# cisco-open/flame

Measured on AMD Instinct MI355X. Metric: aggregated params/sec (device-resident), 1024-client FedAvg @1/2/4/8 GPU, higher is better.
Workload: dtype f32

## Files before the change

### flame_amd/csrc/fedagg.hip

```cpp
#include <hip/hip_runtime.h>
#include <hip/hip_fp16.h>

#include <atomic>
#include <cstdint>
#include <cstdio>
#include <cstring>
#include <cstdarg>
#include <type_traits>

#include "../../include/flame_amd.h"
#include "fastmath.h"

#if defined(__FAST_MATH__) || (defined(__FINITE_MATH_ONLY__) && __FINITE_MATH_ONLY__)
#error "fedagg.hip must not be built with -ffast-math / -ffinite-math-only"
#endif

namespace {

constexpr int kBlock = 256;
#ifndef FLAME_T_CLIENT_UNROLL
#define FLAME_T_CLIENT_UNROLL 8
#endif
constexpr int kClientUnroll = FLAME_T_CLIENT_UNROLL;
#ifndef FLAME_T_CLIENT_UNROLL16
#define FLAME_T_CLIENT_UNROLL16 8
#endif
constexpr int kClientUnroll16 = FLAME_T_CLIENT_UNROLL16;
#ifndef FLAME_T_LO_UNROLL
#define FLAME_T_LO_UNROLL 3
#endif
constexpr int kLoUnroll = FLAME_T_LO_UNROLL;
#ifndef FLAME_T_LO_UNROLL16
#define FLAME_T_LO_UNROLL16 4
#endif
constexpr int kLoUnroll16 = FLAME_T_LO_UNROLL16;
#ifndef FLAME_T_LO_LDS
#define FLAME_T_LO_LDS 65536
#endif
constexpr int kLoLds = FLAME_T_LO_LDS;
#ifndef FLAME_T_LO_WGC
#define FLAME_T_LO_WGC 8
#endif
constexpr int kLoWGC = FLAME_T_LO_WGC;
#ifndef FLAME_T_LO_BURST_MAX_CLIENTS
#define FLAME_T_LO_BURST_MAX_CLIENTS 512
#endif
constexpr int kLoBurstMaxClients = FLAME_T_LO_BURST_MAX_CLIENTS;
constexpr int kLoHeld = kLoWGC > 1 ? kLoWGC * 4096 : 0;
constexpr int kLoDynLds = kLoLds > kLoHeld ? kLoLds - kLoHeld : 0;
#ifndef FLAME_T_LO_MIN_CLIENTS
#define FLAME_T_LO_MIN_CLIENTS 64
#endif
constexpr int kLoMinClients = FLAME_T_LO_MIN_CLIENTS;
#ifndef FLAME_T_LO_MIN_CHUNKS
#define FLAME_T_LO_MIN_CHUNKS 4096
#endif
constexpr int64_t kLoMinChunks = FLAME_T_LO_MIN_CHUNKS;
#ifndef FLAME_T_OPT_WGC
#define FLAME_T_OPT_WGC 4
#endif
constexpr int kOptWGC = FLAME_T_OPT_WGC;
#ifndef FLAME_T_OPT_UNROLL
#define FLAME_T_OPT_UNROLL 3
#endif
constexpr int kOptUnroll = FLAME_T_OPT_UNROLL;
#ifndef FLAME_T_HB
#define FLAME_T_HB 8
#endif
constexpr int kHB = FLAME_T_HB;
#ifndef FLAME_T_HIER_UNROLL16
#define FLAME_T_HIER_UNROLL16 4
#endif
constexpr int kHierUnroll16 = FLAME_T_HIER_UNROLL16;
#ifndef FLAME_T_HBL
#define FLAME_T_HBL 16
#endif
constexpr int kHBL = FLAME_T_HBL;
#ifndef FLAME_T_HIER_LDS_UNROLL16
#define FLAME_T_HIER_LDS_UNROLL16 6
#endif
constexpr int kHierLdsUnroll16 = FLAME_T_HIER_LDS_UNROLL16;
#ifndef FLAME_T_HLDS_MIN_MIDS
#define FLAME_T_HLDS_MIN_MIDS 16
#endif
constexpr int kHLdsMinMids = FLAME_T_HLDS_MIN_MIDS;
#ifndef FLAME_T_HLO_UNROLL
#define FLAME_T_HLO_UNROLL 3
#endif
constexpr int kHLoUnroll = FLAME_T_HLO_UNROLL;
#ifndef FLAME_T_HLO_MIN_CLIENTS
#define FLAME_T_HLO_MIN_CLIENTS 64
#endif
constexpr int kHLoMinClients = FLAME_T_HLO_MIN_CLIENTS;
#ifndef FLAME_T_HLO_MIN_CHUNKS
#define FLAME_T_HLO_MIN_CHUNKS 4096
#endif
constexpr int64_t kHLoMinChunks = FLAME_T_HLO_MIN_CHUNKS;
#ifndef FLAME_T_HLO_LDS_F32
#define FLAME_T_HLO_LDS_F32 65536
#endif
constexpr int kHLoLdsF32 = FLAME_T_HLO_LDS_F32;
#ifndef FLAME_T_HLO_LDS16
#define FLAME_T_HLO_LDS16 53248
#endif
constexpr int kHLoLds16 = FLAME_T_HLO_LDS16;
#ifndef FLAME_T_DYN_UNROLL
#define FLAME_T_DYN_UNROLL 4
#endif
constexpr int kDynUnroll = FLAME_T_DYN_UNROLL;
#ifndef FLAME_T_CHAIN_UNROLL
#define FLAME_T_CHAIN_UNROLL 16
#endif
constexpr int kChainUnroll = FLAME_T_CHAIN_UNROLL;
#ifndef FLAME_T_CHAIN_UNROLL16
#define FLAME_T_CHAIN_UNROLL16 8
#endif
constexpr int kChainUnroll16 = FLAME_T_CHAIN_UNROLL16;
#ifndef FLAME_T_CHAIN_LDS
#define FLAME_T_CHAIN_LDS 53248
#endif
constexpr int kChainLds = FLAME_T_CHAIN_LDS;
#ifndef FLAME_T_BF16_PACKED
#define FLAME_T_BF16_PACKED 1
#endif
constexpr bool kBf16Packed = FLAME_T_BF16_PACKED != 0;
#ifndef FLAME_T_F16_PACKED
#define FLAME_T_F16_PACKED 1
#endif
constexpr bool kF16Packed = FLAME_T_F16_PACKED != 0;
#ifndef FLAME_T_F16_HWROOT
#define FLAME_T_F16_HWROOT 1
#endif
constexpr bool kF16HwRoot = FLAME_T_F16_HWROOT != 0;
#ifndef FLAME_T_F16_NATIVE
#define FLAME_T_F16_NATIVE 1
#endif
constexpr bool kF16Native = FLAME_T_F16_NATIVE != 0;
#ifndef FLAME_T_F16_HSQRT
#define FLAME_T_F16_HSQRT 1
#endif
constexpr bool kF16HalfRoot = FLAME_T_F16_HSQRT != 0;
#ifndef FLAME_T_HALF_ADMIT
#define FLAME_T_HALF_ADMIT 1
#endif
constexpr bool kHalfAdmit = FLAME_T_HALF_ADMIT != 0;
#ifndef FLAME_T_YOGI_SIGN
#define FLAME_T_YOGI_SIGN 1
#endif
constexpr bool kYogiSelect = FLAME_T_YOGI_SIGN != 0;
constexpr int kEwBlock = 256;

thread_local char g_err[512] = "";

int set_err(int code, const char* fmt, ...) {
    va_list ap;
    va_start(ap, fmt);
    vsnprintf(g_err, sizeof(g_err), fmt, ap);
    va_end(ap);
    return code;
}

int check_launch(const char* what) {
    hipError_t e = hipGetLastError();
    if (e != hipSuccess) return set_err(FLAME_EHIP, "%s: %s", what, hipGetErrorString(e));
    g_err[0] = 0;
    return FLAME_OK;
}

__device__ __forceinline__ float bf16_round(float x) {
    return static_cast<float>(static_cast<__bf16>(x));
}
__device__ __forceinline__ float bf16_to_f32(uint16_t b) {
    return __uint_as_float(static_cast<uint32_t>(b) << 16);
}
__device__ __forceinline__ uint16_t f32_to_bf16_exact(float x) {
    return static_cast<uint16_t>(__float_as_uint(x) >> 16);
}
__device__ __forceinline__ float bf16_rnd1(float x) {
    float r;
    asm("v_cvt_pk_bf16_f32 %0, 0, %1" : "=v"(r) : "v"(x));
    return r;
}
using f2 = __attribute__((ext_vector_type(2))) float;
__device__ __forceinline__ f2 bf16_rnd2(f2 x) { return f2{bf16_rnd1(x.x), bf16_rnd1(x.y)}; }
__device__ __forceinline__ f2 splat2(float x) { return f2{x, x}; }
__device__ __forceinline__ float f16_round(float x) {
    asm volatile("" : "+v"(x));
    return static_cast<float>(static_cast<_Float16>(x));
}
__device__ __forceinline__ float f16_to_f32(uint16_t h) {
    _Float16 v;
    __builtin_memcpy(&v, &h, 2);
    return static_cast<float>(v);
}
__device__ __forceinline__ uint16_t f32_to_f16_bits(float x) {
    asm volatile("" : "+v"(x));
    _Float16 v = static_cast<_Float16>(x);
    uint16_t h;
    __builtin_memcpy(&h, &v, 2);
    return h;
}
__device__ __forceinline__ f2 f16_rnd2(f2 x) {
    uint32_t p;
    asm("v_cvt_pk_f16_f32 %0, %1, %2" : "=v"(p) : "v"(x.x), "v"(x.y));
    return f2{f16_to_f32(static_cast<uint16_t>(p)), f16_to_f32(static_cast<uint16_t>(p >> 16))};
}

using h2 = __attribute__((ext_vector_type(2))) _Float16;
using us2 = __attribute__((ext_vector_type(2))) unsigned short;
__device__ __forceinline__ h2 h2_of(uint32_t u) { return __builtin_bit_cast(h2, u); }
__device__ __forceinline__ uint32_t u_of(h2 h) { return __builtin_bit_cast(uint32_t, h); }
__device__ __forceinline__ f2 widen_h2(uint32_t u) {
    const h2 h = h2_of(u);
    return f2{static_cast<float>(h.x), static_cast<float>(h.y)};
}
__device__ __forceinline__ uint32_t smul_h2(float s, uint32_t x, float& lo, float& hi) {
    uint32_t r;
    asm("v_fma_mix_f32 %0, %1, %2, neg(0) op_sel_hi:[0,1,0]" : "=v"(lo) : "s"(s), "v"(x));
    asm("v_fma_mix_f32 %0, %1, %2, neg(0) op_sel:[0,1,0] op_sel_hi:[0,1,0]" : "=v"(hi) : "s"(s), "v"(x));
    asm("v_cvt_pk_f16_f32 %0, %1, %2" : "=v"(r) : "v"(lo), "v"(hi));
    return r;
}
__device__ __forceinline__ uint32_t smul_h2(float s, uint32_t x) {
    float lo, hi;
    return smul_h2(s, x, lo, hi);
}
template <int HI>
__device__ __forceinline__ float div_rn_h(uint32_t x, float den) {
    const float y = flame_fm::rcp_rn(den);
    float q0;
    if constexpr (HI) asm("v_fma_mix_f32 %0, %1, %2, neg(0) op_sel:[0,1,0] op_sel_hi:[0,1,0]" : "=v"(q0) : "v"(y), "v"(x));
    else asm("v_fma_mix_f32 %0, %1, %2, neg(0) op_sel_hi:[0,1,0]" : "=v"(q0) : "v"(y), "v"(x));
    const float a = static_cast<float>(HI ? h2_of(x).y : h2_of(x).x);
    const float rn = __builtin_fmaf(den, q0, -a);
    return __builtin_fmaf(-rn, y, q0);
}
__device__ __forceinline__ uint32_t pk_h2(f2 x) {
    uint32_t r;
    asm("v_cvt_pk_f16_f32 %0, %1, %2" : "=v"(r) : "v"(x.x), "v"(x.y));
    return r;
}
__device__ __forceinline__ h2 sign_h2(h2 x) {
    const h2 z = x + h2{0, 0};
    const h2 big = (z * h2{65504, 65504}) * h2{65504, 65504};
    return __builtin_elementwise_max(__builtin_elementwise_min(big, h2{1, 1}), h2{-1, -1});
}

template <int DT> struct Tr;

template <> struct Tr<FLAME_F32> {
    using T = float; using A = float; static constexpr int EPT = 4;
    __device__ static A ld(T x) { return x; }
    __device__ static T st(A a) { return a; }
    __device__ static A tmp(T v, float r, double) { return __fmul_rn(v, r); }
    __device__ static A mulr(A a, float r, double) { return __fmul_rn(a, r); }
    __device__ static A add(A a, A t) { return __fadd_rn(a, t); }
};
template <> struct Tr<FLAME_BF16> {
    using T = uint16_t; using A = float; static constexpr int EPT = 8;
    __device__ static A ld(T x) { return bf16_to_f32(x); }
    __device__ static T st(A a) { return f32_to_bf16_exact(a); }
    __device__ static A tmp(T v, float r, double) { return bf16_round(__fmul_rn(bf16_to_f32(v), r)); }
// ... 2247 lines not shown
                    for (int j = 0; j < EPT; ++j) {
                        S::op(w[j], X::st(acc[j]), g, static_cast<double>(g), &d[j]);
                        const A t = X::tmp(d[j], rt, 0.0);
                        top[j] = have_top ? X::add(top[j], t) : t;
                    }
                }
                if constexpr (HL) held[u * kBlock + threadIdx.x] = pack<T, EPT>(w);
                else pend[u] = pack<T, EPT>(w);
                if (dp) st_v(dp, pack<T, EPT>(d));
            }
            have_top = true;
            }
            if (!(flags & FLAME_HIER_MID_READONLY)) {
#pragma unroll
                for (int u = 0; u < HB; ++u) {
                    if (u >= nb) break;
                    T* wp = mid_ptr(m0 + u);
                    V16 pv;
                    if constexpr (HL) pv = held[u * kBlock + threadIdx.x];
                    else pv = pend[u];
                    st_v(wp, pv);
                }
            }
        }
        T o[EPT];
#pragma unroll
        for (int j = 0; j < EPT; ++j) o[j] = X::st(top[j]);
        if (sg.top_agg_out) st_v(reinterpret_cast<T*>(sg.top_agg_out) + e0, pack<T, EPT>(o));
        if (flags & FLAME_HIER_TOP_APPLY) {
            T* gp = reinterpret_cast<T*>(sg.top_w) + e0;
            T gw[EPT];
            unpack<T, EPT>(ld_v(gp), gw);
#pragma unroll
            for (int j = 0; j < EPT; ++j) S::op(gw[j], o[j], top_goal, static_cast<double>(top_goal), nullptr);
            st_v(gp, pack<T, EPT>(gw));
        }
        return;
    }
    hier_tail<DT, SYNC>(sg, e0, coff, wrow, drow, crow, mid_ptr, n_mids, n_clients, mid_rates, mid_goal, top_rates,
                        top_goal, flags);
}

template <int DT, int CU, bool SYNC, int HB, bool HL>
__global__ __launch_bounds__(kBlock) void hier_fedbuff_kernel(const flame_hier_segment* __restrict__ segs, int n_segs,
                                                    int n_mids, int n_clients, const uint64_t* __restrict__ mid_w,
                                                    const uint64_t* __restrict__ mid_delta,
                                                    const uint64_t* __restrict__ clients,
                                                    const float* __restrict__ mid_rates,
                                                    const float* __restrict__ mid_goal,
                                                    const float* __restrict__ top_rates, float top_goal,
                                                    unsigned flags) {
    hier_fedbuff_body<DT, CU, SYNC, HB, HL>(segs, n_segs, n_mids, n_clients, mid_w, mid_delta, clients, mid_rates, mid_goal,
                                    top_rates, top_goal, flags);
}

template <int DT, int CU, bool SYNC, int HB, bool HL>
__global__ __launch_bounds__(kBlock) void hier_fedbuff_kernel_argmeta(const ArgMeta meta, int n_segs, int n_mids, int n_clients,
                                                            int o_mid_w, int o_mid_delta, int o_clients,
                                                            int o_mid_rates, int o_mid_goal, int o_top_rates,
                                                            float top_goal, unsigned flags) {
    (void)sizeof(meta);
    const uint64_t* w = (const uint64_t*)__builtin_amdgcn_kernarg_segment_ptr();
    hier_fedbuff_body<DT, CU, SYNC, HB, HL>(reinterpret_cast<const flame_hier_segment*>(w), n_segs, n_mids, n_clients,
                                    w + o_mid_w, o_mid_delta >= 0 ? w + o_mid_delta : nullptr, w + o_clients,
                                    reinterpret_cast<const float*>(w + o_mid_rates),
                                    reinterpret_cast<const float*>(w + o_mid_goal),
                                    reinterpret_cast<const float*>(w + o_top_rates), top_goal, flags);
}
#pragma clang diagnostic pop

template <int DT, int CU, bool VEC>
__device__ __forceinline__ void feddyn_chunk(const flame_dyn_segment& sg, const uint64_t* __restrict__ row,
                                             const uint32_t* __restrict__ sflags, int n_steps, int n_phase1,
                                             float ra32, float rm32, double ra64, double rm64, int64_t e0,
                                             int64_t coff, int64_t hoff) {
    using X = Tr<DT>;
    using T = typename X::T;
    using A = typename X::A;
    constexpr int EPT = X::EPT;
    const int64_t ooff = e0 * static_cast<int64_t>(sizeof(T));
    auto load = [&](uint64_t base, int64_t off, T (&x)[EPT]) {
        const T* p = reinterpret_cast<const T*>(reinterpret_cast<const char*>(base) + off);
        if constexpr (VEC) {
            unpack<T, EPT>(ld_nt(p), x);
        } else {
#pragma unroll
            for (int j = 0; j < EPT; ++j) x[j] = (e0 + j < sg.numel) ? ld1(p + j) : T(0);
        }
    };
    auto store = [&](void* base, int64_t off, const T (&x)[EPT]) {
        T* p = reinterpret_cast<T*>(reinterpret_cast<char*>(base) + off);
        if constexpr (VEC) {
            st_v(p, pack<T, EPT>(x));
        } else {
#pragma unroll
            for (int j = 0; j < EPT; ++j)
                if (e0 + j < sg.numel) st1(p + j, x[j]);
        }
    };
    A avg[EPT], mean[EPT];
    {
        T b[EPT];
        load(reinterpret_cast<uint64_t>(sg.in), ooff, b);
#pragma unroll
        for (int j = 0; j < EPT; ++j) { avg[j] = X::ld(b[j]); mean[j] = A(0); }
    }
#pragma unroll 1
    for (int phase = 0; phase < 2; ++phase) {
        const int end = phase ? n_steps : n_phase1;
#pragma unroll 1
        for (int k = phase ? n_phase1 : 0; k < end; k += CU) {
            const int nb = (end - k < CU) ? end - k : CU;
            T w[CU][EPT], h[CU][EPT];
#pragma unroll
            for (int u = 0; u < CU; ++u) {
                if (u >= nb) break;
                const uint32_t f = sflags[k + u];
                const uint64_t* p = row + static_cast<int64_t>(k + u) * 3;
                if (f & FLAME_DYN_W) load(p[0], coff, w[u]);
                if (f & FLAME_DYN_HIN) load(p[1], hoff, h[u]);
            }
#pragma unroll
            for (int u = 0; u < CU; ++u) {
                if (u >= nb) break;
                const uint32_t f = sflags[k + u];
                if (f & FLAME_DYN_AVG) {
#pragma unroll
                    for (int j = 0; j < EPT; ++j) avg[j] = X::add(avg[j], X::tmp(w[u][j], ra32, ra64));
                }
                if (f & FLAME_DYN_HOUT) {
                    if (f & FLAME_DYN_HIN) {
#pragma unroll
                        for (int j = 0; j < EPT; ++j) h[u][j] = X::st(X::add(X::ld(h[u][j]), X::ld(w[u][j])));
                    } else {
#pragma unroll
                        for (int j = 0; j < EPT; ++j) h[u][j] = w[u][j];
                    }
                    store(reinterpret_cast<void*>(row[static_cast<int64_t>(k + u) * 3 + 2]), hoff, h[u]);
                }
                if (f & FLAME_DYN_MEAN) {
#pragma unroll
                    for (int j = 0; j < EPT; ++j) mean[j] = X::add(mean[j], X::tmp(h[u][j], rm32, rm64));
                }
            }
        }
    }
    T o[EPT], c[EPT];
#pragma unroll
    for (int j = 0; j < EPT; ++j) { o[j] = X::st(avg[j]); c[j] = X::st(X::add(avg[j], mean[j])); }
    store(sg.out, ooff, o);
    store(sg.cld, ooff, c);
}

template <int DT, int CU>
__global__ __launch_bounds__(kBlock) void feddyn_kernel(const flame_dyn_segment* __restrict__ segs, int n_segs,
                                                        const uint64_t* __restrict__ steps,
                                                        const uint32_t* __restrict__ sflags, int n_steps,
                                                        int n_phase1, float ra32, float rm32, double ra64,
                                                        double rm64) {
    using X = Tr<DT>;
    constexpr int EPT = X::EPT;
    const int64_t chunk = xcd_slot(blockIdx.x, gridDim.x);
    const int s = find_segment(segs, n_segs, chunk);
    const flame_dyn_segment sg = segs[s];
    const int64_t e0 = (chunk - sg.chunk_begin) * chunk_elems<DT>() + static_cast<int64_t>(threadIdx.x) * EPT;
    if (e0 >= sg.numel) return;
    const int64_t coff = client_offset<DT>(sg, chunk);
    const int64_t hoff = sg.hist_tile_stride
        ? (chunk - sg.chunk_begin) * sg.hist_tile_stride + static_cast<int64_t>(threadIdx.x) * EPT * static_cast<int64_t>(sizeof(typename X::T))
        : e0 * static_cast<int64_t>(sizeof(typename X::T));
    const uint64_t* row = steps + static_cast<int64_t>(s) * n_steps * 3;
    const bool vec = (e0 + EPT <= sg.numel) && !(sg.flags & FLAME_SEG_UNALIGNED);
    if (vec)
        feddyn_chunk<DT, CU, true>(sg, row, sflags, n_steps, n_phase1, ra32, rm32, ra64, rm64, e0, coff, hoff);
    else
        feddyn_chunk<DT, 1, false>(sg, row, sflags, n_steps, n_phase1, ra32, rm32, ra64, rm64, e0, coff, hoff);
}

__host__ __device__ __forceinline__ uint64_t mix64(uint64_t z) {
    z = (z ^ (z >> 30)) * 0xBF58476D1CE4E5B9ull;
    z = (z ^ (z >> 27)) * 0x94D049BB133111EBull;
    return z ^ (z >> 31);
}

template <int DT>
__global__ __launch_bounds__(kEwBlock) void synth_kernel(void* out, int64_t numel, uint64_t ck, int64_t start, float scale) {
    const int64_t stride = static_cast<int64_t>(gridDim.x) * kEwBlock;
    for (int64_t j = static_cast<int64_t>(blockIdx.x) * kEwBlock + threadIdx.x; j < numel; j += stride) {
        const uint64_t h = mix64(ck + static_cast<uint64_t>(start + j) * 0x9E3779B97F4A7C15ull);
        const int32_t s = static_cast<int32_t>((h & 0xFFFFu) + ((h >> 16) & 0xFFFFu) + ((h >> 32) & 0xFFFFu) + (h >> 48)) - 131070;
        const float x = __fmul_rn(static_cast<float>(s), scale);
        if constexpr (DT == FLAME_F32) st1(reinterpret_cast<float*>(out) + j, x);
        else if constexpr (DT == FLAME_BF16) st1(reinterpret_cast<uint16_t*>(out) + j, f32_to_bf16_exact(bf16_round(x)));
        else st1(reinterpret_cast<uint16_t*>(out) + j, f32_to_f16_bits(x));
    }
}

__device__ __forceinline__ void philox4x32_10(uint32_t (&c)[4], uint32_t k0, uint32_t k1) {
#pragma unroll
    for (int r = 0; r < 10; ++r) {
        const uint64_t p0 = 0xD2511F53ull * c[0], p1 = 0xCD9E8D57ull * c[2];
        const uint32_t n0 = static_cast<uint32_t>(p1 >> 32) ^ c[1] ^ k0;
        const uint32_t n2 = static_cast<uint32_t>(p0 >> 32) ^ c[3] ^ k1;
        c[0] = n0; c[1] = static_cast<uint32_t>(p1); c[2] = n2; c[3] = static_cast<uint32_t>(p0);
        k0 += 0x9E3779B9u; k1 += 0xBB67AE85u;
    }
}

__device__ __forceinline__ float noise_neg2ln(float u) {
    const uint32_t bits = __float_as_uint(u);
    int e = static_cast<int>(bits >> 23) - 127;
    float m = __uint_as_float((bits & 0x7FFFFFu) | 0x3F800000u);
    if (m > 0x1.6a09e6p+0f) { m = __fmul_rn(m, 0.5f); e += 1; }
    const float f = __fadd_rn(m, -1.0f);
    const float s = __fdiv_rn(f, __fadd_rn(f, 2.0f));
    const float z = __fmul_rn(s, s);
    float p = 0x1.745d18p-4f;
    p = __fadd_rn(__fmul_rn(p, z), 0x1.c71c72p-4f);
    p = __fadd_rn(__fmul_rn(p, z), 0x1.24924ap-3f);
    p = __fadd_rn(__fmul_rn(p, z), 0x1.99999ap-3f);
    p = __fadd_rn(__fmul_rn(p, z), 0x1.555556p-2f);
    p = __fmul_rn(p, z);
    const float t = __fadd_rn(s, s);
    const float lg = __fadd_rn(t, __fmul_rn(t, p));
    const float ef = static_cast<float>(e);
    const float ln = __fadd_rn(__fmul_rn(ef, 0x1.62e4p-1f), __fadd_rn(lg, __fmul_rn(ef, 0x1.7f7d1cp-20f)));
    return __fmul_rn(-2.0f, ln);
}

__device__ __forceinline__ void noise_sincos(uint32_t k, float& co, float& si) {
    const uint32_t o = k >> 21, j = k & 0x1FFFFFu;
    const uint32_t jj = (o & 1u) ? 0x200000u - j : j;
    const float phi = __fmul_rn(static_cast<float>(jj), 0x1.921fb6p-22f);
    const float z = __fmul_rn(phi, phi);
    float ps = 0x1.71de3ap-19f;
    ps = __fadd_rn(__fmul_rn(ps, z), -0x1.a01a02p-13f);
    ps = __fadd_rn(__fmul_rn(ps, z), 0x1.111112p-7f);
    ps = __fadd_rn(__fmul_rn(ps, z), -0x1.555556p-3f);
    const float s = __fadd_rn(phi, __fmul_rn(__fmul_rn(phi, z), ps));
    float pc = -0x1.27e4fcp-22f;
    pc = __fadd_rn(__fmul_rn(pc, z), 0x1.a01a02p-16f);
    pc = __fadd_rn(__fmul_rn(pc, z), -0x1.6c16c2p-10f);
    pc = __fadd_rn(__fmul_rn(pc, z), 0x1.555556p-5f);
    pc = __fadd_rn(__fmul_rn(pc, z), -0x1p-1f);
    const float c = __fadd_rn(1.0f, __fmul_rn(z, pc));
    const bool swap = ((o + 1u) >> 1) & 1u, cneg = ((o + 2u) >> 2) & 1u, sneg = o >> 2;
    const float c0 = swap ? s : c, s0 = swap ? c : s;
    co = __uint_as_float(__float_as_uint(c0) ^ (cneg ? 0x80000000u : 0u));
    si = __uint_as_float(__float_as_uint(s0) ^ (sneg ? 0x80000000u : 0u));
}

__device__ __forceinline__ void noise_pair(uint32_t xu, uint32_t xk, float& ze, float& zo) {
    const uint64_t v = 2ull * xu + 1ull;
    const float hi = static_cast<float>(static_cast<uint32_t>(v >> 17));
    const float lo = static_cast<float>(static_cast<uint32_t>(v & 0x1FFFFu));
    const float u = __fmul_rn(__fadd_rn(__fmul_rn(hi, 131072.0f), lo), 0x1p-33f);
    const float r = __builtin_sqrtf(noise_neg2ln(u));
    float co, si;
    noise_sincos(xk >> 8, co, si);
    ze = __fmul_rn(r, co);
    zo = __fmul_rn(r, si);
}

__device__ __forceinline__ void noise_block(uint32_t k0, uint32_t k1, uint32_t round, uint32_t stream, uint64_t b,
                                            float (&z)[4]) {
    uint32_t c[4] = {static_cast<uint32_t>(b), static_cast<uint32_t>(b >> 32), stream, round};
    philox4x32_10(c, k0, k1);
    noise_pair(c[0], c[1], z[0], z[1]);
    noise_pair(c[2], c[3], z[2], z[3]);
}

template <int DT>
__device__ __forceinline__ typename Tr<DT>::T noise_value(float z, float std32, double std64) {
    if constexpr (DT == FLAME_F64) return __dmul_rn(static_cast<double>(z), std64);
    else if constexpr (DT == FLAME_F32) return __fmul_rn(z, std32);
    else if constexpr (DT == FLAME_BF16) return f32_to_bf16_exact(bf16_round(__fmul_rn(z, std32)));
    else return f32_to_f16_bits(__fmul_rn(z, std32));
}

template <int DT>
__global__ __launch_bounds__(kBlock) void noise_fill_kernel(const flame_segment* __restrict__ segs, int n_segs,
                                                          const uint32_t* __restrict__ streams,
                                                          const int64_t* __restrict__ starts, uint32_t k0, uint32_t k1,
                                                          uint32_t round, float std32, double std64) {
    using T = typename Tr<DT>::T;
    constexpr int EPT = Tr<DT>::EPT;
    const int64_t chunk = blockIdx.x;
    const int s = find_segment(segs, n_segs, chunk);
    const flame_segment sg = segs[s];
    const int64_t e0 = (chunk - sg.chunk_begin) * chunk_elems<DT>() + static_cast<int64_t>(threadIdx.x) * EPT;
    if (e0 >= sg.numel) return;
    const uint32_t stream = streams[s];
    const uint64_t start = static_cast<uint64_t>(starts[s]);
    const uint64_t g0 = start + static_cast<uint64_t>(e0);
    T* op = reinterpret_cast<T*>(sg.out) + e0;
    float z[4];
    if ((e0 + EPT <= sg.numel) && !(sg.flags & FLAME_SEG_UNALIGNED) && !(start & 3u)) {
        T x[EPT];
        if constexpr (EPT >= 4) {
#pragma unroll
            for (int q = 0; q < EPT / 4; ++q) {
                noise_block(k0, k1, round, stream, (g0 >> 2) + q, z);
#pragma unroll
                for (int j = 0; j < 4; ++j) x[4 * q + j] = noise_value<DT>(z[j], std32, std64);
            }
        } else {
            noise_block(k0, k1, round, stream, g0 >> 2, z);
            const bool up = g0 & 2u;
            x[0] = noise_value<DT>(up ? z[2] : z[0], std32, std64);
            x[1] = noise_value<DT>(up ? z[3] : z[1], std32, std64);
        }
        st_v(op, pack<T, EPT>(x));
        return;
    }
    uint64_t have = ~0ull;
    for (int j = 0; j < EPT; ++j) {
        if (e0 + j >= sg.numel) break;
        const uint64_t g = g0 + static_cast<uint64_t>(j);
        if ((g >> 2) != have) {
            have = g >> 2;
            noise_block(k0, k1, round, stream, have, z);
        }
        const uint32_t l = static_cast<uint32_t>(g) & 3u;
        const float zl = l == 0 ? z[0] : l == 1 ? z[1] : l == 2 ? z[2] : z[3];
        st1(op + j, noise_value<DT>(zl, std32, std64));
// ... 867 lines not shown
                               n_segs, cl, n_clients, rates32, step_end, flags, b1, omb1, b2, omb2, eta, tau);
        });
    });
    if (!known) return set_err(FLAME_ENOTSUP, "%s: dtype %d not supported (f32, bf16, f16)", who, dtype);
    return launched(BR_CHAIN + dtype * 3 + variant, who);
}

int flame_fedopt_reduce_adapt_f64(int variant, unsigned flags, const flame_segment* segs, int32_t n_segs,
                                  int64_t n_chunks, const void* const* clients, int32_t n_clients,
                                  const double* rates64, double b1, double omb1, double b2, double omb2, double eta,
                                  double tau, void* stream) {
    const char* const who = "flame_fedopt_reduce_adapt_f64";
    if (int rc = validate(segs, n_segs, n_chunks, n_clients, clients)) return rc;
    if (n_clients > 0 && !rates64) return set_err(FLAME_EINVAL, "rate array is NULL");
    if (int rc = check_variant(who, variant)) return rc;
    if (int rc = check_flags(who, flags, kOptFlags)) return rc;
    hipStream_t st = reinterpret_cast<hipStream_t>(stream);
    const dim3 grid(static_cast<unsigned>(n_chunks)), block(kBlock);
    auto cl = reinterpret_cast<const uint64_t*>(clients);
    const Hyper64 h{b1, omb1, b2, omb2, eta, tau};
    dispatch_variant(variant, [&](auto vr) {
        hipLaunchKernelGGL((fedopt_kernel_f64<decltype(vr)::value, kClientUnroll>), grid, block, 0, st, segs, n_segs, cl,
                           n_clients, rates64, flags, h, n_chunks);
    });
    return launched(BR_OPT_F64 + variant, who);
}

int flame_fedopt_chain_f64(int variant, unsigned flags, const flame_segment* segs, int32_t n_segs, int64_t n_chunks,
                           const void* const* clients, int32_t n_clients, const double* rates64,
                           const uint8_t* step_end, double b1, double omb1, double b2, double omb2, double eta,
                           double tau, void* stream) {
    const char* const who = "flame_fedopt_chain_f64";
    if (int rc = validate(segs, n_segs, n_chunks, n_clients, clients)) return rc;
    if (n_clients < 1 || !rates64 || !step_end)
        return set_err(FLAME_EINVAL, "%s: needs >= 1 client, a rate array and a step_end array", who);
    if (int rc = check_variant(who, variant)) return rc;
    if (int rc = check_flags(who, flags, FLAME_OPT_STATE_ZERO)) return rc;
    hipStream_t st = reinterpret_cast<hipStream_t>(stream);
    const dim3 grid(static_cast<unsigned>(n_chunks)), block(kBlock);
    auto cl = reinterpret_cast<const uint64_t*>(clients);
    const Hyper64 h{b1, omb1, b2, omb2, eta, tau};
    dispatch_variant(variant, [&](auto vr) {
        hipLaunchKernelGGL((fedopt_chain_kernel_f64<decltype(vr)::value, kClientUnroll>), grid, block, 0, st, segs, n_segs,
                           cl, n_clients, rates64, step_end, flags, h);
    });
    return launched(BR_CHAIN_F64 + variant, who);
}

int flame_fedopt_reduce_adapt_argmeta(int dtype, int variant, unsigned flags, const void* host_meta,
                                      int64_t meta_bytes, int32_t n_segs, int64_t n_chunks, int32_t n_clients,
                                      int64_t off_clients, int64_t off_r32, float b1, float omb1, float b2,
                                      float omb2, float eta, float tau, void* stream) {
    const char* const who = "flame_fedopt_reduce_adapt_argmeta";
    ArgMeta m;
    if (int rc = load_argmeta(who, host_meta, meta_bytes, m)) return rc;
    if (n_segs <= 0 || n_clients < 0) return set_err(FLAME_EINVAL, "%s: n_segs <= 0 or n_clients < 0", who);
    if (int rc = check_chunks(n_chunks)) return rc;
    if (int rc = check_flags(who, flags, kOptFlags)) return rc;
    if (int rc = check_variant(who, variant)) return rc;
    if (static_cast<int64_t>(n_segs) * static_cast<int64_t>(sizeof(flame_segment)) > meta_bytes ||
        !inside(meta_bytes, off_clients, static_cast<int64_t>(n_segs) * n_clients * 8) ||
        (n_clients > 0 && !inside(meta_bytes, off_r32, static_cast<int64_t>(n_clients) * 4)))
        return set_err(FLAME_EINVAL, "%s: a table lies outside the metadata block", who);
    const OptArgMeta src{&m, static_cast<int>(off_clients / 8), n_clients > 0 ? static_cast<int>(off_r32 / 8) : -1};
    return launch_opt(who, dtype, variant, flags, src, n_segs, n_clients, n_chunks, Hyper32{b1, omb1, b2, omb2, eta, tau},
                      stream);
}

int flame_fedbuff_scale_add(int dtype, const flame_segment* segs, int32_t n_segs, int64_t n_chunks, int64_t goal,
                            void* stream) {
    if (int rc = validate(segs, n_segs, n_chunks, 0, nullptr)) return rc;
    if (goal == 0) return set_err(FLAME_EINVAL, "agg_goal must be nonzero");
    hipStream_t st = reinterpret_cast<hipStream_t>(stream);
    const dim3 grid(static_cast<unsigned>(n_chunks)), block(kEwBlock);
    const float gf = static_cast<float>(goal);
    const double gd = static_cast<double>(goal);
    const bool known = dispatch<FLAME_F32, FLAME_F64, FLAME_BF16, FLAME_F16>(dtype, [&](auto dt) {
        hipLaunchKernelGGL((scale_add_kernel<decltype(dt)::value>), grid, block, 0, st, segs, n_segs, gf, gd);
    });
    if (!known)
        return set_err(FLAME_ENOTSUP, "flame_fedbuff_scale_add: dtype %d not supported (integer tensors raise in the reference)", dtype);
    return launched(BR_SA + dtype, "flame_fedbuff_scale_add");
}

int flame_hier_fedbuff(int dtype, unsigned flags, const flame_hier_segment* segs, int32_t n_segs, int64_t n_chunks,
                       int32_t n_mids, int32_t n_clients, const void* const* mid_w, const void* const* mid_delta,
                       const void* const* clients, const float* mid_rates, const float* mid_goal,
                       const float* top_rates, float top_goal, void* stream) {
    const char* const who = "flame_hier_fedbuff";
    if (!segs || n_segs <= 0) return set_err(FLAME_EINVAL, "segment table is NULL or n_segs <= 0");
    if (int rc = check_chunks(n_chunks)) return rc;
    if (n_mids < 1 || n_clients < 1) return set_err(FLAME_EINVAL, "%s: need >= 1 middle and >= 1 arrival per middle", who);
    if (!mid_w || !clients || !mid_rates || !mid_goal || !top_rates) return set_err(FLAME_EINVAL, "%s: NULL table", who);
    if (int rc = check_hier_flags(who, flags, top_goal)) return rc;
    const HierTables src{segs, reinterpret_cast<const uint64_t*>(mid_w), reinterpret_cast<const uint64_t*>(mid_delta),
                         reinterpret_cast<const uint64_t*>(clients), mid_rates, mid_goal, top_rates};
    return launch_hier(who, dtype, flags, src, n_segs, n_chunks, n_mids, n_clients, top_goal, stream);
}

int flame_hier_fedbuff_argmeta(int dtype, unsigned flags, const void* host_meta, int64_t meta_bytes, int32_t n_segs,
                               int64_t n_chunks, int32_t n_mids, int32_t n_clients, int64_t off_mid_w,
                               int64_t off_mid_delta, int64_t off_clients, int64_t off_mid_rates,
                               int64_t off_mid_goal, int64_t off_top_rates, float top_goal, void* stream) {
    const char* const who = "flame_hier_fedbuff_argmeta";
    ArgMeta m;
    if (int rc = load_argmeta(who, host_meta, meta_bytes, m)) return rc;
    if (n_segs <= 0) return set_err(FLAME_EINVAL, "segment table is empty");
    if (int rc = check_chunks(n_chunks)) return rc;
    if (n_mids < 1 || n_clients < 1) return set_err(FLAME_EINVAL, "%s: need >= 1 middle and >= 1 arrival per middle", who);
    if (int rc = check_hier_flags(who, flags, top_goal)) return rc;
    const int64_t S = n_segs, M = n_mids, C = n_clients;
    if (S * static_cast<int64_t>(sizeof(flame_hier_segment)) > meta_bytes || !inside(meta_bytes, off_mid_w, S * M * 8) ||
        (off_mid_delta >= 0 && !inside(meta_bytes, off_mid_delta, S * M * 8)) ||
        !inside(meta_bytes, off_clients, S * M * C * 8) || !inside(meta_bytes, off_mid_rates, M * C * 4) ||
        !inside(meta_bytes, off_mid_goal, M * 4) || !inside(meta_bytes, off_top_rates, M * 4))
        return set_err(FLAME_EINVAL, "%s: a table lies outside the metadata block", who);
    const HierArgMeta src{&m, static_cast<int>(off_mid_w / 8), off_mid_delta >= 0 ? static_cast<int>(off_mid_delta / 8) : -1,
                          static_cast<int>(off_clients / 8), static_cast<int>(off_mid_rates / 8),
                          static_cast<int>(off_mid_goal / 8), static_cast<int>(off_top_rates / 8)};
    return launch_hier(who, dtype, flags, src, n_segs, n_chunks, n_mids, n_clients, top_goal, stream);
}

int flame_hier_resident_per_cu(int dtype, unsigned flags, int32_t n_mids) {
    if (n_mids < 1) return -set_err(FLAME_EINVAL, "flame_hier_resident_per_cu: n_mids < 1");
    HierPick p = pick_hier(flags, n_mids, 0, 0);
    p.lo = false;
    const void* f = nullptr;
    const bool known = dispatch_hier(dtype, p, [&](auto inst) {
        using I = decltype(inst);
        f = reinterpret_cast<const void*>(hier_fedbuff_kernel<I::DT, I::CU, I::SYNC, I::HB, I::HL>);
    });
    if (!known)
        return -set_err(FLAME_ENOTSUP, "flame_hier_resident_per_cu: dtype %d not supported (f32, bf16, f16)", dtype);
    int blocks = 0;
    const hipError_t e = hipOccupancyMaxActiveBlocksPerMultiprocessor(&blocks, f, kBlock, 0);
    if (e != hipSuccess) return -set_err(FLAME_EHIP, "hipOccupancyMaxActiveBlocksPerMultiprocessor: %s", hipGetErrorString(e));
    return blocks < 1 ? 1 : blocks;
}

int flame_feddyn_round(int dtype, const flame_dyn_segment* segs, int32_t n_segs, int64_t n_chunks,
                       const void* const* steps, const uint32_t* step_flags, int32_t n_steps, int32_t n_phase1,
                       double rate_avg, double rate_mean, void* stream) {
    if (!segs || n_segs <= 0) return set_err(FLAME_EINVAL, "segment table is NULL or n_segs <= 0");
    if (int rc = check_chunks(n_chunks)) return rc;
    if (n_steps < 1 || !steps) return set_err(FLAME_EINVAL, "flame_feddyn_round: empty step program");
    if (n_steps > 0 && !step_flags) return set_err(FLAME_EINVAL, "flame_feddyn_round: step flag array is NULL");
    if (n_phase1 < 0 || n_phase1 > n_steps)
        return set_err(FLAME_EINVAL, "flame_feddyn_round: n_phase1 %d outside [0, %d]", n_phase1, n_steps);
    hipStream_t st = reinterpret_cast<hipStream_t>(stream);
    const dim3 grid(static_cast<unsigned>(n_chunks)), block(kBlock);
    auto sp = reinterpret_cast<const uint64_t*>(steps);
    const float ra32 = static_cast<float>(rate_avg), rm32 = static_cast<float>(rate_mean);
    const bool known = dispatch<FLAME_F32, FLAME_BF16, FLAME_F16, FLAME_F64>(dtype, [&](auto dt) {
        hipLaunchKernelGGL((feddyn_kernel<decltype(dt)::value, kDynUnroll>), grid, block, 0, st, segs, n_segs, sp, step_flags,
                           n_steps, n_phase1, ra32, rm32, rate_avg, rate_mean);
    });
    if (!known) return set_err(FLAME_ENOTSUP, "flame_feddyn_round: dtype %d not supported (f32, bf16, f16, f64)", dtype);
    return launched(BR_DYN + dtype, "flame_feddyn_round");
}

int flame_host_register(void* host, uint64_t nbytes) {
    if (!host || nbytes == 0) return set_err(FLAME_EINVAL, "flame_host_register: empty range");
    hipError_t e = hipHostRegister(host, static_cast<size_t>(nbytes), hipHostRegisterMapped | hipHostRegisterPortable);
    if (e != hipSuccess) return set_err(FLAME_EHIP, "hipHostRegister: %s", hipGetErrorString(e));
    return FLAME_OK;
}

int flame_host_unregister(void* host) {
    if (!host) return set_err(FLAME_EINVAL, "flame_host_unregister: NULL");
    hipError_t e = hipHostUnregister(host);
    if (e != hipSuccess) return set_err(FLAME_EHIP, "hipHostUnregister: %s", hipGetErrorString(e));
    return FLAME_OK;
}

int flame_host_device_pointer(void* host, void** device) {
    if (!host || !device) return set_err(FLAME_EINVAL, "flame_host_device_pointer: NULL");
    hipError_t e = hipHostGetDevicePointer(device, host, 0);
    if (e != hipSuccess) return set_err(FLAME_EHIP, "hipHostGetDevicePointer: %s", hipGetErrorString(e));
    return FLAME_OK;
}

int flame_synth_fill(int dtype, void* out, int64_t numel, uint64_t seed, uint64_t stream_id, int64_t start,
                     float scale, void* stream) {
    if (numel < 0 || (numel > 0 && !out)) return set_err(FLAME_EINVAL, "flame_synth_fill: bad buffer");
    if (numel == 0) return FLAME_OK;
    const uint64_t ck = mix64((seed * 0x9E3779B97F4A7C15ull) ^ ((stream_id + 1ull) * 0xD1B54A32D192ED03ull));
    hipStream_t st = reinterpret_cast<hipStream_t>(stream);
    int64_t blocks = (numel + kEwBlock - 1) / kEwBlock;
    if (blocks > 8192) blocks = 8192;
    const dim3 grid(static_cast<unsigned>(blocks)), block(kEwBlock);
    const bool known = dispatch<FLAME_F32, FLAME_BF16, FLAME_F16>(dtype, [&](auto dt) {
        hipLaunchKernelGGL(synth_kernel<decltype(dt)::value>, grid, block, 0, st, out, numel, ck, start, scale);
    });
    if (!known) return set_err(FLAME_ENOTSUP, "flame_synth_fill: dtype %d not supported", dtype);
    return check_launch("flame_synth_fill");
}

int flame_noise_fill(int dtype, const flame_segment* segs, int32_t n_segs, int64_t n_chunks, const uint32_t* streams,
                     const int64_t* starts, uint64_t seed, uint32_t round, double std, void* stream) {
    const char* const who = "flame_noise_fill";
    if (int rc = need_segs(who, segs, n_segs)) return rc;
    if (n_chunks <= 0 || n_chunks > 0x7FFFFFFFll)
        return set_err(FLAME_EINVAL, "%s: n_chunks out of range: %lld", who, (long long)n_chunks);
    if (dtype == FLAME_I64 || dtype == FLAME_I32)
        return set_err(FLAME_ENOTSUP, "%s: float dtypes only (integer and bool tensors get no noise), got dtype %d", who, dtype);
    if (dtype != FLAME_F32 && dtype != FLAME_BF16 && dtype != FLAME_F16 && dtype != FLAME_F64)
        return set_err(FLAME_ENOTSUP, "%s: unknown dtype %d", who, dtype);
    if (!(std >= 0.0) || std > 1.7976931348623157e308)
        return set_err(FLAME_EINVAL, "%s: std must be a finite number >= 0, got %g", who, std);
    if (dtype != FLAME_F64 && std >= 0x1.ffffffp127)
        return set_err(FLAME_EINVAL, "%s: std %g rounds to an infinite fp32", who, std);
    if (!streams || !starts) return set_err(FLAME_EINVAL, "%s: the streams / starts array is NULL", who);
    hipStream_t st = reinterpret_cast<hipStream_t>(stream);
    const dim3 grid(static_cast<unsigned>(n_chunks)), block(kBlock);
    const uint32_t k0 = static_cast<uint32_t>(seed), k1 = static_cast<uint32_t>(seed >> 32);
    const float std32 = dtype == FLAME_F64 ? 0.f : static_cast<float>(std);
    dispatch<FLAME_F32, FLAME_BF16, FLAME_F16, FLAME_F64>(dtype, [&](auto dt) {
        hipLaunchKernelGGL((noise_fill_kernel<decltype(dt)::value>), grid, block, 0, st, segs, n_segs, streams, starts, k0,
                           k1, round, std32, std);
    });
    return check_launch(who);
}

static int ew_check(const flame_ew_op* prog, int32_t n_ops, void* const* bufs, int32_t n_bufs, int64_t numel);

int flame_elementwise(const flame_ew_op* prog, int32_t n_ops, void* const* bufs, int32_t n_bufs, int64_t numel,
                      void* stream) {
    if (n_bufs < 0 || n_bufs > FLAME_EW_MAX_BUFS || (n_bufs > 0 && !bufs))
        return set_err(FLAME_EINVAL, "flame_elementwise: n_bufs %d outside [0, %d] or NULL table", n_bufs, FLAME_EW_MAX_BUFS);
    const int rc = ew_check(prog, n_ops, bufs, n_bufs, numel);
    if (rc != FLAME_OK) return rc;
    if (numel == 0 || n_ops == 0) return FLAME_OK;
    EwArgs a{};
    for (int32_t k = 0; k < n_ops; ++k) a.ops[k] = prog[k];
    for (int32_t k = 0; k < n_bufs; ++k) a.bufs[k] = bufs[k];
    a.numel = numel;
    a.n_ops = n_ops;
    int64_t blocks = (numel + kEwBlock - 1) / kEwBlock;
    if (blocks > 4096) blocks = 4096;
    hipLaunchKernelGGL(ew_kernel, dim3(static_cast<unsigned>(blocks)), dim3(kEwBlock), 0,
                       reinterpret_cast<hipStream_t>(stream), a);
    return launched(BR_EW, "flame_elementwise");
}

int flame_elementwise_segments(const flame_ew_op* prog, int32_t n_ops, void* const* table, int32_t n_bufs,
                               const int64_t* seg_end, int32_t n_segs, int64_t numel, void* stream) {
    if (n_bufs < 0 || n_bufs > FLAME_EW_MAX_BUFS)
        return set_err(FLAME_EINVAL, "flame_elementwise_segments: n_bufs %d outside [0, %d]", n_bufs, FLAME_EW_MAX_BUFS);
    if (n_segs <= 0 || !table || !seg_end)
        return set_err(FLAME_EINVAL, "flame_elementwise_segments: n_segs <= 0 or a NULL table");
    const int rc = ew_check(prog, n_ops, nullptr, n_bufs, numel);
    if (rc != FLAME_OK) return rc;
    if (numel == 0 || n_ops == 0) return FLAME_OK;
    EwArgs a{};
    for (int32_t k = 0; k < n_ops; ++k) a.ops[k] = prog[k];
    a.table = table;
    a.seg_end = seg_end;
    a.numel = numel;
    a.n_ops = n_ops;
    a.n_segs = n_segs;
    a.n_bufs = n_bufs;
    int64_t blocks = (numel + kEwBlock - 1) / kEwBlock;
    if (blocks > 4096) blocks = 4096;
    hipLaunchKernelGGL(ew_kernel, dim3(static_cast<unsigned>(blocks)), dim3(kEwBlock), 0,
                       reinterpret_cast<hipStream_t>(stream), a);
    return launched(BR_EW_SEG, "flame_elementwise_segments");
}

static int ew_check(const flame_ew_op* prog, int32_t n_ops, void* const* bufs, int32_t n_bufs, int64_t numel) {
    if (n_ops < 0 || n_ops > FLAME_EW_MAX_OPS || (n_ops > 0 && !prog))
        return set_err(FLAME_EINVAL, "flame_elementwise: n_ops %d outside [0, %d] or NULL program", n_ops, FLAME_EW_MAX_OPS);
    if (numel < 0) return set_err(FLAME_EINVAL, "flame_elementwise: numel < 0");
    int rdt[FLAME_EW_MAX_REGS];
    for (int k = 0; k < FLAME_EW_MAX_REGS; ++k) rdt[k] = -1;
    auto reg = [](int x) { return x >= 0 && x < FLAME_EW_MAX_REGS; };
    for (int32_t k = 0; k < n_ops; ++k) {
        const flame_ew_op& o = prog[k];
        const int dt = o.dtype;
        if (dt < FLAME_F32 || dt > FLAME_BOOL) return set_err(FLAME_EINVAL, "flame_elementwise: op %d: dtype %d", k, dt);
        auto bad = [&](const char* why) { return set_err(FLAME_EINVAL, "flame_elementwise: op %d (%d): %s", k, o.op, why); };
        switch (o.op) {
        case FLAME_EW_LOAD:
            if (!reg(o.dst) || o.a < 0 || o.a >= n_bufs || (bufs && numel > 0 && !bufs[o.a])) return bad("bad register or buffer");
            rdt[o.dst] = dt;
            break;
        case FLAME_EW_STORE:
            if (!reg(o.b) || o.a < 0 || o.a >= n_bufs || (bufs && numel > 0 && !bufs[o.a])) return bad("bad register or buffer");
            if (rdt[o.b] != dt) return bad("stored register is not of the buffer's dtype");
            break;
        case FLAME_EW_ZERO:
            if (!reg(o.dst)) return bad("bad register");
            rdt[o.dst] = dt;
            break;
        case FLAME_EW_CAST:
            if (!reg(o.dst) || !reg(o.a) || rdt[o.a] < 0 || rdt[o.a] != o.b) return bad("source register undefined or not of dtype b");
            rdt[o.dst] = dt;
            break;
        case FLAME_EW_ADD: case FLAME_EW_SUB: case FLAME_EW_MUL: case FLAME_EW_DIV:
            if (!reg(o.dst) || !reg(o.a) || !reg(o.b) || rdt[o.a] != dt || rdt[o.b] != dt) return bad("operand not of the op's dtype");
            if (o.op == FLAME_EW_DIV && !ew_float(dt)) return bad("division in an integer dtype");
            if (dt == FLAME_BOOL && o.op == FLAME_EW_SUB) return bad("subtraction in bool");
            rdt[o.dst] = dt;
            break;
        case FLAME_EW_ADD_S: case FLAME_EW_MUL_S: case FLAME_EW_SQUARE: case FLAME_EW_SIGN: case FLAME_EW_SQRT:
            if (!reg(o.dst) || !reg(o.a) || rdt[o.a] != dt) return bad("operand not of the op's dtype");
            if (o.op == FLAME_EW_SQRT && !ew_float(dt)) return bad("sqrt in an integer dtype");
            if (dt == FLAME_BOOL && (o.op == FLAME_EW_ADD_S || o.op == FLAME_EW_MUL_S))
// ... 85 lines not shown
```

Before: 1803 billion.

## Add double-buffered steady-state FedDyn path with nontemporal loads and buffer stores

Adds a specialised FedDyn kernel path for programs where every step carries the full steady flag set. In that path each lane issues 16-byte nontemporal loads for the next batch of client weights and history while it consumes the current batch, and writes history and outputs with raw buffer stores marked nontemporal. The aim is to hide global-memory latency and reduce cache pollution in the client loop. In exchange, every block first scans the step flags to detect the steady case, register pressure rises from the doubled load buffers, and the generic path is kept as a fallback. This only touches the FedDyn round, not the FedAvg aggregation that the benchmark measures.

```diff
diff --git a/flame_amd/csrc/fedagg.hip b/flame_amd/csrc/fedagg.hip
--- a/flame_amd/csrc/fedagg.hip
+++ b/flame_amd/csrc/fedagg.hip
@@ -108,6 +108,14 @@
 #define FLAME_T_DYN_UNROLL 4
 #endif
 constexpr int kDynUnroll = FLAME_T_DYN_UNROLL;
+#ifndef FLAME_T_DYN_PIPE
+#define FLAME_T_DYN_PIPE 2
+#endif
+constexpr int kDynPipe = FLAME_T_DYN_PIPE;
+#ifndef FLAME_T_DYN_LDS
+#define FLAME_T_DYN_LDS 0
+#endif
+constexpr int kDynLds = FLAME_T_DYN_LDS;
 #ifndef FLAME_T_CHAIN_UNROLL
 #define FLAME_T_CHAIN_UNROLL 16
 #endif
@@ -2661,7 +2669,102 @@
     store(sg.cld, ooff, c);
 }
 
-template <int DT, int CU>
+__device__ __forceinline__ u4 ld_nt4(const void* p) { return __builtin_nontemporal_load(G(reinterpret_cast<const u4*>(p))); }
+__device__ __forceinline__ void st_chunk(void* chunk, uint32_t lane_off, const u4& x) {
+    constexpr int kRawDword3 = 0x00020000;
+    constexpr int kSc0 = 1, kNt = 2, kSc1 = 16;
+    const __amdgpu_buffer_rsrc_t r = __builtin_amdgcn_make_buffer_rsrc(chunk, 0, FLAME_TILE_BYTES, kRawDword3);
+    __builtin_amdgcn_raw_buffer_store_b128(x, r, static_cast<int>(lane_off), 0, kSc0 | kSc1 | kNt);
+}
+constexpr uint32_t kDynSteady = FLAME_DYN_W | FLAME_DYN_HIN | FLAME_DYN_AVG | FLAME_DYN_HOUT | FLAME_DYN_MEAN;
+
+template <int DT, int B>
+__device__ __forceinline__ void feddyn_steady(const flame_dyn_segment& sg, const uint64_t* __restrict__ row,
+                                              int n_steps, float ra32, float rm32, double ra64, double rm64,
+                                              int64_t ochunk, int64_t hchunk, uint32_t lane, int64_t coff) {
+    using X = Tr<DT>;
+    using T = typename X::T;
+    using A = typename X::A;
+    constexpr int EPT = X::EPT;
+    static_assert(sizeof(T) * EPT == 16, "lane vector is 16 bytes");
+    using kptr = const __attribute__((address_space(4))) uint64_t*;
+    const kptr steps = reinterpret_cast<kptr>(reinterpret_cast<uintptr_t>(row));
+    const int64_t hoff = hchunk + lane;
+    auto issue = [&](int k0, u4 (&w)[B], u4 (&h)[B]) {
+#pragma unroll
+        for (int u = 0; u < B; ++u) {
+            const kptr p = steps + static_cast<int64_t>(k0 + u) * 3;
+            w[u] = ld_nt4(reinterpret_cast<const char*>(p[0]) + coff);
+            h[u] = ld_nt4(reinterpret_cast<const char*>(p[1]) + hoff);
+        }
+    };
+    A avg[EPT], mean[EPT];
+    auto step = [&](int k, const u4& wv, const u4& hv) {
+        T w[EPT], h[EPT];
+        __builtin_memcpy(w, &wv, 16);
+        __builtin_memcpy(h, &hv, 16);
+#pragma unroll
+        for (int j = 0; j < EPT; ++j) avg[j] = X::add(avg[j], X::tmp(w[j], ra32, ra64));
+#pragma unroll
+        for (int j = 0; j < EPT; ++j) h[j] = X::st(X::add(X::ld(h[j]), X::ld(w[j])));
+        u4 hn;
+        __builtin_memcpy(&hn, h, 16);
+        st_chunk(reinterpret_cast<char*>(steps[static_cast<int64_t>(k) * 3 + 2]) + hchunk, lane, hn);
+#pragma unroll
+        for (int j = 0; j < EPT; ++j) mean[j] = X::add(mean[j], X::tmp(h[j], rm32, rm64));
+    };
+    auto consume = [&](int k0, const u4 (&w)[B], const u4 (&h)[B]) {
+#pragma unroll
+        for (int u = 0; u < B; ++u) step(k0 + u, w[u], h[u]);
+    };
+    u4 w0[B], h0[B], w1[B], h1[B];
+    const u4 base = ld_nt4(reinterpret_cast<const char*>(sg.in) + ochunk + lane);
+    const int nfull = n_steps / B;
+    if (nfull > 0) issue(0, w0, h0);
+    {
+        T b[EPT];
+        __builtin_memcpy(b, &base, 16);
+#pragma unroll
+        for (int j = 0; j < EPT; ++j) { avg[j] = X::ld(b[j]); mean[j] = A(0); }
+    }
+    if (nfull > 0) {
+        int kb = 0;
+#pragma unroll 1
+        for (;;) {
+            if (kb + 1 == nfull) { consume(kb * B, w0, h0); break; }
+            issue((kb + 1) * B, w1, h1);
+            consume(kb * B, w0, h0);
+            ++kb;
+            if (kb + 1 == nfull) { consume(kb * B, w1, h1); break; }
+            issue((kb + 1) * B, w0, h0);
+            consume(kb * B, w1, h1);
+            ++kb;
+        }
+    }
+#pragma unroll 1
+    for (int k = nfull * B; k < n_steps; ++k) {
+        const kptr p = steps + static_cast<int64_t>(k) * 3;
+        const u4 w = ld_nt4(reinterpret_cast<const char*>(p[0]) + coff);
+        const u4 h = ld_nt4(reinterpret_cast<const char*>(p[1]) + hoff);
+        step(k, w, h);
+    }
+    T o[EPT], c[EPT];
+#pragma unroll
+    for (int j = 0; j < EPT; ++j) { o[j] = X::st(avg[j]); c[j] = X::st(X::add(avg[j], mean[j])); }
+    u4 ov, cv;
+    __builtin_memcpy(&ov, o, 16);
+    __builtin_memcpy(&cv, c, 16);
+    st_chunk(reinterpret_cast<char*>(sg.out) + ochunk, lane, ov);
+    st_chunk(reinterpret_cast<char*>(sg.cld) + ochunk, lane, cv);
+}
+
+__device__ __forceinline__ bool feddyn_program_steady(const uint32_t* __restrict__ sflags, int n_steps) {
+    bool ok = true;
+    for (int i = threadIdx.x & 63; i < n_steps; i += 64) ok &= ld1(sflags + i) == kDynSteady;
+    return __all(ok);
+}
+
+template <int DT, int CU, int B>
 __global__ __launch_bounds__(kBlock) void feddyn_kernel(const flame_dyn_segment* __restrict__ segs, int n_segs,
                                                         const uint64_t* __restrict__ steps,
                                                         const uint32_t* __restrict__ sflags, int n_steps,
@@ -2669,6 +2772,7 @@
                                                         double rm64) {
     using X = Tr<DT>;
     constexpr int EPT = X::EPT;
+    const bool steady = B > 0 && n_phase1 == n_steps && feddyn_program_steady(sflags, n_steps);
     const int64_t chunk = xcd_slot(blockIdx.x, gridDim.x);
     const int s = find_segment(segs, n_segs, chunk);
     const flame_dyn_segment sg = segs[s];
@@ -2680,6 +2784,16 @@
         : e0 * static_cast<int64_t>(sizeof(typename X::T));
     const uint64_t* row = steps + static_cast<int64_t>(s) * n_steps * 3;
     const bool vec = (e0 + EPT <= sg.numel) && !(sg.flags & FLAME_SEG_UNALIGNED);
+    if constexpr (B > 0) {
+        const bool whole = (chunk - sg.chunk_begin + 1) * chunk_elems<DT>() <= sg.numel;
+        if (steady && whole && !(sg.flags & FLAME_SEG_UNALIGNED)) {
+            const int64_t c = chunk - sg.chunk_begin;
+            feddyn_steady<DT, B>(sg, row, n_steps, ra32, rm32, ra64, rm64, c * FLAME_TILE_BYTES,
+                                 c * (sg.hist_tile_stride ? sg.hist_tile_stride : FLAME_TILE_BYTES),
+                                 threadIdx.x * 16u, coff);
+            return;
+        }
+    }
     if (vec)
         feddyn_chunk<DT, CU, true>(sg, row, sflags, n_steps, n_phase1, ra32, rm32, ra64, rm64, e0, coff, hoff);
     else
@@ -3853,7 +3967,7 @@
     auto sp = reinterpret_cast<const uint64_t*>(steps);
     const float ra32 = static_cast<float>(rate_avg), rm32 = static_cast<float>(rate_mean);
     const bool known = dispatch<FLAME_F32, FLAME_BF16, FLAME_F16, FLAME_F64>(dtype, [&](auto dt) {
-        hipLaunchKernelGGL((feddyn_kernel<decltype(dt)::value, kDynUnroll>), grid, block, 0, st, segs, n_segs, sp, step_flags,
+        hipLaunchKernelGGL((feddyn_kernel<decltype(dt)::value, kDynUnroll, kDynPipe>), grid, block, kDynLds, st, segs, n_segs, sp, step_flags,
                            n_steps, n_phase1, ra32, rm32, rate_avg, rate_mean);
     });
     if (!known) return set_err(FLAME_ENOTSUP, "flame_feddyn_round: dtype %d not supported (f32, bf16, f16, f64)", dtype);
```

Result: no change. 1803 billion (median of 2 runs) (-0.0%).
